# grayhong/self-diagnosing-gan

Measured on AMD Instinct MI355X. Metric: images/sec (G+D step), higher is better.
Workload: dtype f32

## Files before the change

include/diagan_conv_x3.h:

```cpp
#ifndef DIAGAN_CONV_X3_H
#define DIAGAN_CONV_X3_H

#include <stdint.h>

#ifdef __cplusplus
extern "C" {
#endif

int diagan_conv_gemm_set_x3_resident(int mode);
int diagan_conv_gemm_get_x3_resident(void);
int diagan_conv_gemm_last_x3_form(void);
int diagan_conv_gemm_x3_resident_ok(int B, int Hi, int Wi, int Ci, int Ho, int Wo, int Co, int R, int S, int sy, int dr, int off, int up,
                                    int Kp, int pro_mode);

#ifdef __cplusplus
}
#endif
#endif
```

self-diagnosing-gan_amd/csrc/conv_wgrad.hip:

```cpp
#include "conv_common.h"
#include "switches.h"
#include <stdlib.h>
#include <type_traits>


namespace diagan {
bool wgrad_wino_supported(int Hi, int Wi, int Ci, int Ho, int Wo, int Co, int R, int S, int sy, int dr, int off, int up,
                          int Kp);
int wgrad_wino_splits(int B, int Ho, int Wo, int Ci, int Co);
int launch_wgrad_wino(WgradArgs a, int splits, int segments, hipStream_t st);
int launch_wgrad_wino_batched(const WgradArgs* jobs, const int* splits, const int* segments, int n, hipStream_t st);
int wgrad_wino_batch_max();
bool wgrad_x3_takes(const WgradArgs& a, bool x3_on);
int launch_wgrad_x3(const WgradArgs& a, int splits, hipStream_t st);
void wgrad_x3_set(int on);


template <int BNn, int BNk, int PRO, bool P2>
__device__ __forceinline__ void conv_wgrad_body(const WgradArgs& a, const int bid, const int nblk) {
  constexpr int BK = 32;
  constexpr int TM = BNn / 64, TN = BNk / 64;
  constexpr int AC = BNn / 4, BC = BNk / 4;
  constexpr int AJ = BK * AC / 256, BJ = BK * BC / 256;
  constexpr int APR = 256 / AC, BPR = 256 / BC;
  constexpr bool BOX = PRO == PRO_BOX || PRO == PRO_BOX_RELU;
  constexpr int BQ = BOX ? 4 : 1;
  __shared__ __attribute__((aligned(16))) float As[2][BK * BNn];
  __shared__ __attribute__((aligned(16))) float Bs[2][BK * BNk];

  const ConvGeom& g = a.g;
  const int tid = threadIdx.x, lane = tid & 63, wave = tid >> 6;
  const int wm = wave >> 1, wn = wave & 1;
  const int tiles_k = (g.Kp + BNk - 1) / BNk;
  const int logical = xcd_remap(bid, nblk);
  const int split = logical / a.tiles, tile = logical - split * a.tiles;
  const int n0 = (tile / tiles_k) * BNn, k0 = (tile % tiles_k) * BNk;
  const int seg = split / a.splits_per_seg, sub = split - seg * a.splits_per_seg;
  const int step0 = seg * a.seg_steps + sub * a.steps_per_split;
  const int step1 = min(step0 + a.steps_per_split, (seg + 1) * a.seg_steps);

  const int pro_mode = PRO >= 0 ? PRO : a.pro_mode;
  const int ac = tid % AC, ap = tid / AC;
  const int an = n0 + ac * 4;
  const unsigned a_kill = an < g.Co ? 0u : 0x80000000u;
  const int bc = tid % BC, bp = tid / BC;
  const int kf = k0 + bc * 4;
  const int tap = kf / g.Ci, kc = kf - tap * g.Ci;
  const int kr = tap / g.S, ks = tap - kr * g.S;
  const bool b_ok = kf < g.K;
  const int dyo = kr * g.dr + g.off, dxo = ks * g.dr + g.off;
  const int upm = g.up - 1, ush = g.up >> 1;
  const int pstep = (g.Ci * 4) >> ush;
  const int img_bytes = BOX ? (g.Hi - 1) * (g.Wi - 1) * g.Ci * 4 : g.Hi * g.Wi * g.Ci * 4;
  const unsigned ylim = (unsigned)g.Hi << ush, xlim = (unsigned)g.Wi << ush;

  const __amdgpu_buffer_rsrc_t ysrc = __builtin_amdgcn_make_buffer_rsrc(
      const_cast<float*>(a.dy), 0, (int)((unsigned)a.M * g.Co * 4u), 0x00020000);
  const __amdgpu_buffer_rsrc_t xsrc = __builtin_amdgcn_make_buffer_rsrc(
      const_cast<float*>(a.x), 0, (int)((unsigned)g.B * (BOX ? (g.Hi - 1) * (g.Wi - 1) : g.Hi * g.Wi) * g.Ci * 4u), 0x00020000);
  const bool affine = pro_mode == PRO_AFFINE_RELU || pro_mode == PRO_AFFINE;
  f32x4 psc = {1.f, 1.f, 1.f, 1.f}, psh = {0.f, 0.f, 0.f, 0.f};
  if (affine && b_ok) {
    psc = *reinterpret_cast<const f32x4*>(a.pro_scale + kc);
    psh = *reinterpret_cast<const f32x4*>(a.pro_shift + kc);
  }
  int pb[BJ], py[BJ], px[BJ];
#pragma unroll
  for (int j = 0; j < BJ; ++j) {
    const int m = step0 * BK + bp + BPR * j;
    const unsigned t = fdiv((unsigned)m, a.dWo);
    px[j] = m - (int)t * g.Wo;
    const unsigned b = fdiv(t, a.dHo);
    py[j] = (int)t - (int)b * g.Ho;
    pb[j] = (int)b;
  }
  int mstep = step0 * BK;
  unsigned xoff[BJ];
  const unsigned xstep = (unsigned)BK * g.Ci * 4u;
#pragma unroll
  for (int j = 0; j < BJ; ++j)
    xoff[j] = (unsigned)((step0 * BK + bp + BPR * j + dyo * g.Wi + dxo) * g.Ci * 4 + kc * 4);
  unsigned aoff[AJ];
#pragma unroll
  for (int j = 0; j < AJ; ++j) aoff[j] = (((unsigned)(step0 * BK + ap + APR * j)) * g.Co + an) * 4u;
  const unsigned astep = (unsigned)BK * g.Co * 4u;
  f32x4 ra[AJ], rb[BJ * BQ];
  unsigned bmask = 0;
  const bool bias_tile = a.bias_off >= 0 && k0 == 0;
  f32x4 bacc = {0.f, 0.f, 0.f, 0.f};
  auto load_piece = [&](int p) {
    if (p < AJ) {
      ra[p] = __builtin_bit_cast(f32x4, __builtin_amdgcn_raw_buffer_load_b128(ysrc, aoff[p] | a_kill, 0, 0));
      aoff[p] += astep;
      return;
    }
    const int j = p - AJ;
    if (j == 0) bmask = 0;
    if (!BOX && P2 && a.same) {
// ... 444 lines not shown
  DG_REQUIRE(table_dev && n_layers > 0 && total_blocks > 0 && total_blocks < (1L << 31), "wgrad_finish_batched: bad args");
  static_assert(sizeof(WgFinish) == 128, "descriptor layout");
  const WgFinish* tab = (const WgFinish*)table_dev;
  hipStream_t st = (hipStream_t)stream;
  hipLaunchKernelGGL(wgrad_finish_a_kernel, dim3((unsigned)total_blocks), dim3(256), 0, st, tab, n_layers);
  if (any_sn) {
    hipLaunchKernelGGL(wgrad_finish_dot_kernel, dim3(n_layers), dim3(256), 0, st, tab);
    hipLaunchKernelGGL(wgrad_finish_b_kernel, dim3((unsigned)total_blocks), dim3(256), 0, st, tab, n_layers);
  }
  return check_launch("wgrad_finish_batched");
}

static void wgrad_tile(int Co, int Kp, int* bn, int* bk) {
  *bn = Co <= 64 ? 64 : 128;
  *bk = Kp <= 64 ? 64 : 128;
  if (*bn == 128 && *bk == 64) *bn = 64;
}

static void wgrad_gemm_fields(WgradArgs& a, int* bn, int* bk, bool* p2) {
  const ConvGeom& g = a.g;
  wgrad_tile(g.Co, g.Kp, bn, bk);
  a.tiles = cdiv(g.Co, *bn) * cdiv(g.Kp, *bk);
  a.same = (g.Hi == g.Ho && g.Wi == g.Wo && g.sy == 1 && g.up == 1) ? 1 : 0;
  *p2 = (g.Ho & (g.Ho - 1)) == 0 && (g.Wo & (g.Wo - 1)) == 0;
  a.lgW = a.lgHW = 0;
  while ((1 << a.lgW) < g.Wo) ++a.lgW;
  while ((1 << a.lgHW) < g.Ho * g.Wo) ++a.lgHW;
}

static int wgrad_fill_args(WgradArgs& a, const float* dy, const float* x, float* slab, int splits, int segments,
                           int64_t slab_stride, int64_t bias_off, const float* pro_scale, const float* pro_shift, int pro_mode, int B,
                           int Hi, int Wi, int Ci, int Ho, int Wo, int Co, int R, int S, int sy, int dr, int off, int up, int Kp) {
  DG_REQUIRE(dy && x && slab, "conv_wgrad: null tensor");
  DG_REQUIRE(B > 0 && Hi > 0 && Wi > 0 && Ho > 0 && Wo > 0 && R > 0 && S > 0, "conv_wgrad: bad dims");
  DG_REQUIRE(Ci > 0 && (Ci & 3) == 0 && Co > 0 && (Co & 3) == 0, "conv_wgrad: Ci=%d, Co=%d must be multiples of 4", Ci, Co);
  DG_REQUIRE(up == 1 || up == 2, "conv_wgrad: up=%d unsupported", up);
  DG_REQUIRE(dr == 1 || dr == -1, "conv_wgrad: dr must be +-1");
  DG_REQUIRE(Kp % 32 == 0 && Kp >= R * S * Ci, "conv_wgrad: bad Kp=%d", Kp);
  DG_REQUIRE(splits >= 1, "conv_wgrad: splits=%d", splits);
  DG_REQUIRE(pro_mode >= 0 && pro_mode <= PRO_BOX_RELU, "conv_wgrad: bad pro_mode %d", pro_mode);
  DG_REQUIRE(!(pro_mode == PRO_BOX || pro_mode == PRO_BOX_RELU) || (up == 1 && dr == 1 && Hi >= 2 && Wi >= 2),
             "conv_wgrad: the box-sum loader (pro_mode 5 / 6) gathers forward geometries without up-sampling");
  DG_REQUIRE(!(pro_mode == PRO_AFFINE_RELU || pro_mode == PRO_AFFINE) || (pro_scale && pro_shift),
             "conv_wgrad: affine prologue needs scale/shift");
  DG_REQUIRE(slab_stride >= (int64_t)Co * Kp && (bias_off < 0 || bias_off + Co <= slab_stride),
             "conv_wgrad: slab_stride=%ld too small for Co*Kp=%ld (+bias)", (long)slab_stride, (long)Co * Kp);
  DG_REQUIRE((long)Co * Kp * 4 < (1L << 31), "conv_wgrad: weight tensor must be smaller than 2 GiB");
  DG_REQUIRE((long)B * Ho * Wo * Co * 4 < (1L << 31) && (long)B * Hi * Wi * Ci * 4 < (1L << 31),
             "conv_wgrad: tensors must be smaller than 2 GiB (32-bit buffer offsets)");
  a.dy = dy; a.x = x; a.slab = slab; a.pro_scale = pro_scale; a.pro_shift = pro_shift; a.pro_mode = pro_mode;
  a.M = B * Ho * Wo;
  a.g = ConvGeom{B, Hi, Wi, Ci, Ho, Wo, Co, R, S, sy, dr, off, up, R * S * Ci, Kp};
  a.dWo = make_fastdiv((unsigned)Wo);
  a.dHo = make_fastdiv((unsigned)Ho);
  a.adv_b = 32 / (Ho * Wo);
  a.adv_y = (32 % (Ho * Wo)) / Wo;
  a.adv_x = (32 % (Ho * Wo)) % Wo;
  const int total_steps = cdiv(a.M, 32);
  DG_REQUIRE(segments >= 1 && splits % segments == 0, "conv_wgrad: splits=%d not a multiple of segments=%d", splits, segments);
  DG_REQUIRE(segments == 1 || (a.M % (32 * segments)) == 0, "conv_wgrad: %d pixels do not split into %d segments of whole K-steps", a.M, segments);
  a.seg_steps = cdiv(total_steps, segments);
  a.splits_per_seg = splits / segments;
  a.steps_per_split = cdiv(a.seg_steps, a.splits_per_seg);
  a.slab_stride = slab_stride;
  a.bias_off = bias_off;
  return DIAGAN_OK;
}

DIAGAN_API int diagan_conv_wgrad(const float* dy, const float* x, float* slab, int splits, int segments,
                                 int64_t slab_stride, int64_t bias_off, const float* pro_scale, const float* pro_shift, int pro_mode, int B,
                                 int Hi, int Wi, int Ci, int Ho, int Wo, int Co, int R, int S, int sy,
                                 int dr, int off, int up, int Kp, void* stream) {
  WgradArgs a;
  const int rc = wgrad_fill_args(a, dy, x, slab, splits, segments, slab_stride, bias_off, pro_scale, pro_shift, pro_mode, B, Hi, Wi, Ci,
                                 Ho, Wo, Co, R, S, sy, dr, off, up, Kp);
  if (rc != DIAGAN_OK) return rc;
  hipStream_t st = (hipStream_t)stream;
  if (diagan_conv_wgrad_uses_wino(Hi, Wi, Ci, Ho, Wo, Co, R, S, sy, dr, off, up, Kp))
    return launch_wgrad_wino(a, splits, segments, st);
  int bn, bk;
  bool p2;
  wgrad_gemm_fields(a, &bn, &bk, &p2);
  if (bn == 128 && bk == 128 && wgrad_x3_takes(a, diagan_conv_gemm_get_x3b() != 0)) return launch_wgrad_x3(a, splits, st);
  const dim3 grid(a.tiles * splits);
#define DG_WG(BN_, PRO_) do { if (p2) hipLaunchKernelGGL((conv_wgrad_kernel<BN_, 128, PRO_, true>), grid, dim3(256), 0, st, a); \
                              else hipLaunchKernelGGL((conv_wgrad_kernel<BN_, 128, PRO_, false>), grid, dim3(256), 0, st, a); } while (0)
#define DG_WG_ALL(BN_) switch (pro_mode) { \
      case PRO_NONE: DG_WG(BN_, PRO_NONE); break; \
      case PRO_RELU: DG_WG(BN_, PRO_RELU); break; \
      case PRO_AFFINE_RELU: DG_WG(BN_, PRO_AFFINE_RELU); break; \
      case PRO_LRELU: DG_WG(BN_, PRO_LRELU); break; \
      case PRO_BOX: DG_WG(BN_, PRO_BOX); break; \
      case PRO_BOX_RELU: DG_WG(BN_, PRO_BOX_RELU); break; \
      default: DG_WG(BN_, PRO_AFFINE); break; }
  if (bn == 64 && bk == 64) {
    DG_REQUIRE(pro_mode <= PRO_AFFINE, "conv_wgrad: no box-sum loader on the 64 x 64 tile (Kp <= 64)");
    hipLaunchKernelGGL((conv_wgrad_kernel<64, 64>), grid, dim3(256), 0, st, a);
  } else if (bn == 64) {
    DG_WG_ALL(64)
  } else {
    DG_WG_ALL(128)
  }
#undef DG_WG_ALL
#undef DG_WG
  return check_launch("conv_wgrad");
}

struct diagan_wgrad_job {
  const float* dy;
  const float* x;
  float* slab;
  const float* pro_scale;
  const float* pro_shift;
  int64_t slab_stride, bias_off;
  int32_t splits, segments, pro_mode, B, Hi, Wi, Ci, Ho, Wo, Co, R, S, sy, dr, off, up, Kp, pad_;
};
static_assert(sizeof(diagan_wgrad_job) == 128, "diagan_wgrad_job layout");
DIAGAN_API int diagan_conv_wgrad_batch_class(int Hi, int Wi, int Ci, int Ho, int Wo, int Co, int R, int S, int sy, int dr, int off,
                                             int up, int Kp, int pro_mode) {
  if (diagan_conv_wgrad_uses_wino(Hi, Wi, Ci, Ho, Wo, Co, R, S, sy, dr, off, up, Kp)) return 100 + pro_mode;
  int bn, bk;
  wgrad_tile(Co, Kp, &bn, &bk);
  if (bn == 64 && bk == 64) return pro_mode >= PRO_BOX ? 0 : 1000;
  if (pro_mode != PRO_NONE && pro_mode != PRO_RELU && pro_mode != PRO_BOX && pro_mode != PRO_BOX_RELU) return 0;
  const bool p2 = (Ho & (Ho - 1)) == 0 && (Wo & (Wo - 1)) == 0;
  return 2000 + (bn == 128 ? 100 : 0) + 2 * pro_mode + (p2 ? 1 : 0);
}

template <int BN_, int BK_, int PRO_, bool P2_>
static void launch_wgrad_gemm_batched(const WgradBatchArgs& b, int wgs, hipStream_t st) {
  hipLaunchKernelGGL((conv_wgrad_batched_kernel<BN_, BK_, PRO_, P2_>), dim3(wgs), dim3(256), 0, st, b);
}

DIAGAN_API int diagan_conv_wgrad_batched(const diagan_wgrad_job* jobs, int n, void* stream) {
  DG_REQUIRE(jobs && n >= 1 && n <= WG_BATCH_MAX, "conv_wgrad_batched: 1 .. %d jobs", WG_BATCH_MAX);
  WgradArgs a[WG_BATCH_MAX];
  int splits[WG_BATCH_MAX], segments[WG_BATCH_MAX], cls = -1;
  for (int j = 0; j < n; ++j) {
    const diagan_wgrad_job& q = jobs[j];
    const int c = diagan_conv_wgrad_batch_class(q.Hi, q.Wi, q.Ci, q.Ho, q.Wo, q.Co, q.R, q.S, q.sy, q.dr, q.off, q.up, q.Kp, q.pro_mode);
    DG_REQUIRE(c != 0 && (cls < 0 || c == cls), "conv_wgrad_batched: job %d has batch class %d, the launch's is %d "
               "(diagan_conv_wgrad_batch_class: equal non-zero classes share a launch)", j, c, cls);
    cls = c;
    const int rc = wgrad_fill_args(a[j], q.dy, q.x, q.slab, q.splits, q.segments, q.slab_stride, q.bias_off, q.pro_scale, q.pro_shift,
                                   q.pro_mode, q.B, q.Hi, q.Wi, q.Ci, q.Ho, q.Wo, q.Co, q.R, q.S, q.sy, q.dr, q.off, q.up, q.Kp);
    if (rc != DIAGAN_OK) return rc;
    splits[j] = q.splits;
    segments[j] = q.segments;
  }
  hipStream_t st = (hipStream_t)stream;
  if (cls < 1000) return launch_wgrad_wino_batched(a, splits, segments, n, st);
  WgradBatchArgs b;
  b.n = n;
  int wgs = 0, bn = 0, bk = 0;
  bool p2 = false;
  for (int j = 0; j < n; ++j) {
    wgrad_gemm_fields(a[j], &bn, &bk, &p2);
    b.a[j] = a[j];
    b.blk0[j] = wgs;
    b.cnt[j] = a[j].tiles * splits[j];
    wgs += (b.cnt[j] + 7) & ~7;
  }
  for (int j = n; j < WG_BATCH_MAX; ++j) b.blk0[j] = wgs, b.cnt[j] = 0;
  const int pro = jobs[0].pro_mode;
  if (cls == 1000) {
    launch_wgrad_gemm_batched<64, 64, -1, false>(b, wgs, st);
    return check_launch("conv_wgrad_batched");
  }
#define DG_WGB(BN_, PRO_) do { if (p2) launch_wgrad_gemm_batched<BN_, 128, PRO_, true>(b, wgs, st); \
                               else launch_wgrad_gemm_batched<BN_, 128, PRO_, false>(b, wgs, st); } while (0)
#define DG_WGB_ALL(BN_) switch (pro) { \
      case PRO_NONE: DG_WGB(BN_, PRO_NONE); break; \
      case PRO_RELU: DG_WGB(BN_, PRO_RELU); break; \
      case PRO_BOX: DG_WGB(BN_, PRO_BOX); break; \
      default: DG_WGB(BN_, PRO_BOX_RELU); break; }
  if (bn == 128) {
    DG_WGB_ALL(128)
  } else {
    DG_WGB_ALL(64)
  }
#undef DG_WGB_ALL
#undef DG_WGB
  return check_launch("conv_wgrad_batched");
}
DIAGAN_API int diagan_conv_wgrad_batch_max(void) { return WG_BATCH_MAX; }

DIAGAN_API int diagan_conv_wgrad_uses_wino(int Hi, int Wi, int Ci, int Ho, int Wo, int Co, int R, int S, int sy, int dr,
                                           int off, int up, int Kp) {
  return kWino.get(-1, diagan_conv_gemm_get_wino()) && kWinoWgrad.env() &&
         wgrad_wino_supported(Hi, Wi, Ci, Ho, Wo, Co, R, S, sy, dr, off, up, Kp);
}

DIAGAN_API int diagan_conv_wgrad_uses_x3(int B, int Hi, int Wi, int Ci, int Ho, int Wo, int Co, int R, int S, int sy, int dr, int off,
                                         int up, int Kp, int pro_mode, int64_t bias_off) {
  if (B <= 0 || Ho <= 0 || Wo <= 0 || diagan_conv_wgrad_uses_wino(Hi, Wi, Ci, Ho, Wo, Co, R, S, sy, dr, off, up, Kp)) return 0;
  int bn, bk;
  wgrad_tile(Co, Kp, &bn, &bk);
  if (bn != 128 || bk != 128) return 0;
  WgradArgs a;
  a.pro_mode = pro_mode; a.bias_off = bias_off; a.M = B * Ho * Wo;
  a.g = ConvGeom{B, Hi, Wi, Ci, Ho, Wo, Co, R, S, sy, dr, off, up, R * S * Ci, Kp};
  return wgrad_x3_takes(a, diagan_conv_gemm_get_x3b() != 0) ? 1 : 0;
}
DIAGAN_API int diagan_conv_wgrad_set_x3(int on) {
  wgrad_x3_set(on);
  return DIAGAN_OK;
}

DIAGAN_API int diagan_conv_wgrad_splits_geom(int B, int Hi, int Wi, int Ci, int Ho, int Wo, int Co, int R, int S, int sy,
                                             int dr, int off, int up, int Kp) {
  if (diagan_conv_wgrad_uses_wino(Hi, Wi, Ci, Ho, Wo, Co, R, S, sy, dr, off, up, Kp))
    return wgrad_wino_splits(B, Ho, Wo, Ci, Co);
  return diagan_conv_wgrad_splits(B * Ho * Wo, Co, Kp);
}

DIAGAN_API int diagan_conv_wgrad_splits(int M, int Co, int Kp) {
  int bn, bk;
  wgrad_tile(Co, Kp, &bn, &bk);
  const int tiles = cdiv(Co, bn) * cdiv(Kp, bk);
  const int total_steps = cdiv(M, 32);
  const int min_steps = kWgradMinSteps.env();
  const double fixed = kWgradFixed.env();
  int smax = total_steps / min_steps;
  if (smax > 256) smax = 256;
  int splits = 1;
  double best = 1e30;
  const int slots = 512;
  for (int s = 1; s <= smax; ++s) {
    const double t = (double)cdiv(tiles * s, slots) * ((double)total_steps / s + fixed);
    if (t < best * 0.995) { best = t; splits = s; }
  }
  if (splits < 1) splits = 1;
  if (splits > 256) splits = 256;
  return splits;
}

DIAGAN_API int diagan_wgrad_reduce(const float* slab, int splits, int64_t n_elem, float* out, int accumulate,
                                   const float* w, double* dot_partials, void* stream) {
  DG_REQUIRE(slab && out && splits >= 1 && n_elem > 0 && (n_elem & 3) == 0, "wgrad_reduce: bad args");
  const long n4 = n_elem / 4;
  hipLaunchKernelGGL(wgrad_reduce_kernel, dim3(cdiv(n4, 256)), dim3(256), 0, (hipStream_t)stream, slab,
                     splits, n4, out, accumulate, w, dot_partials);
  return check_launch("wgrad_reduce");
}
```

self-diagnosing-gan_amd/csrc/conv_wgrad_x3.hip:

```cpp
#include "conv_common.h"
#include "switches.h"
#include "wino_weights.h"
#include <stdlib.h>

namespace diagan {

constexpr int WX_ROW = 40;
constexpr int WX_PLANE = 128 * WX_ROW;
constexpr int WX_LDS_BYTES = 6 * WX_PLANE * 2;

typedef __bf16 wx_bf16x8 __attribute__((ext_vector_type(8)));

template <bool NOPAD, bool TWO = false>
__global__ __launch_bounds__(256, 2) void conv_wgrad_x3_kernel(const WgradArgs a) {
  extern __shared__ __attribute__((aligned(16))) unsigned short lds[];
  const ConvGeom& g = a.g;
  const int tid = threadIdx.x, lane = tid & 63, wave = __builtin_amdgcn_readfirstlane(tid >> 6);
  const int wm = wave >> 1, wn = wave & 1;
  const int tiles_k = g.Kp >> 7;
  const int logical = xcd_remap(blockIdx.x, gridDim.x);
  const int split = logical / a.tiles, tile = logical - split * a.tiles;
  const int n0 = (tile / tiles_k) * 128, k0 = (tile % tiles_k) * 128;
  const int seg = split / a.splits_per_seg, sub = split - seg * a.splits_per_seg;
  const int step0 = seg * a.seg_steps + sub * a.steps_per_split;
  const int step1 = min(step0 + a.steps_per_split, (seg + 1) * a.seg_steps);

  const int pq = tid & 7, lc = tid >> 3;
  const __amdgpu_buffer_rsrc_t ysrc = __builtin_amdgcn_make_buffer_rsrc(
      const_cast<float*>(a.dy), 0, (int)((unsigned)a.M * g.Co * 4u), 0x00020000);
  const __amdgpu_buffer_rsrc_t xsrc = __builtin_amdgcn_make_buffer_rsrc(
      const_cast<float*>(a.x), 0, (int)((unsigned)g.B * g.Hi * g.Wi * g.Ci * 4u), 0x00020000);
  unsigned aoff = (((unsigned)(step0 * 32 + 4 * pq)) * g.Co + n0 + 4 * lc) * 4u;
  const unsigned astep = 32u * g.Co * 4u;
  const int arow = g.Co * 4;
  const int kf = k0 + 4 * lc;
  const int tap = kf / g.Ci, kc = kf - tap * g.Ci;
  const int kr = tap / g.S, ks = tap - kr * g.S;
  const bool b_ok = kf < g.K;
  const int dyo = kr * g.dr + g.off, dxo = ks * g.dr + g.off;
  const int cb = g.Ci * 4;
  int pb, py, px;
  {
    const int m = step0 * 32 + 4 * pq;
    const unsigned t = fdiv((unsigned)m, a.dWo);
    px = m - (int)t * g.Wo;
    const unsigned b = fdiv(t, a.dHo);
    py = (int)t - (int)b * g.Ho;
    pb = (int)b;
  }
  f32x4 ra[4], rb[4];
  auto load_step = [&]() __attribute__((always_inline)) {
#pragma unroll
    for (int j = 0; j < 4; ++j)
      ra[j] = __builtin_bit_cast(f32x4, __builtin_amdgcn_raw_buffer_load_b128(ysrc, aoff + (unsigned)(j * arow), 0, 0));
    aoff += astep;
    int x = px, y = py, b = pb;
#pragma unroll
    for (int j = 0; j < 4; ++j) {
      const int iy = y * g.sy + dyo, ix = x * g.sy + dxo;
      bool ok = b_ok && b < g.B;
      if (!NOPAD) ok = ok && (unsigned)iy < (unsigned)g.Hi && (unsigned)ix < (unsigned)g.Wi;
      const unsigned off = (unsigned)(((b * g.Hi + iy) * g.Wi + ix) * cb + kc * 4) | (ok ? 0u : 0x80000000u);
      rb[j] = __builtin_bit_cast(f32x4, __builtin_amdgcn_raw_buffer_load_b128(xsrc, off, 0, 0));
      if (j < 3) {
        ++x;
        const int cx = x >= g.Wo ? 1 : 0;
        x = cx ? 0 : x;
        y += cx;
        const int cy = y >= g.Ho ? 1 : 0;
        y = cy ? 0 : y;
        b += cy;
      }
    }
    {
      int x2 = px + a.adv_x, y2 = py + a.adv_y, b2 = pb + a.adv_b;
      const int cx = x2 >= g.Wo ? 1 : 0;
      x2 -= cx ? g.Wo : 0;
      y2 += cx;
      const int cy = y2 >= g.Ho ? 1 : 0;
      y2 -= cy ? g.Ho : 0;
      b2 += cy;
      px = x2; py = y2; pb = b2;
    }
  };
  const int sto = (4 * lc) * WX_ROW + 4 * pq;
  auto store_step = [&]() __attribute__((always_inline)) {
#pragma unroll
    for (int e = 0; e < 4; ++e) {
      u32x2 p0, p1, p2;
      x3_split(f32x4{ra[0][e], ra[1][e], ra[2][e], ra[3][e]}, p0, p1, p2);
      unsigned short* st = lds + sto + e * WX_ROW;
      *reinterpret_cast<u32x2*>(st) = p0;
      *reinterpret_cast<u32x2*>(st + WX_PLANE) = p1;
      if (!TWO) *reinterpret_cast<u32x2*>(st + 2 * WX_PLANE) = p2;
      x3_split(f32x4{rb[0][e], rb[1][e], rb[2][e], rb[3][e]}, p0, p1, p2);
      *reinterpret_cast<u32x2*>(st + 3 * WX_PLANE) = p0;
      *reinterpret_cast<u32x2*>(st + 4 * WX_PLANE) = p1;
      if (!TWO) *reinterpret_cast<u32x2*>(st + 5 * WX_PLANE) = p2;
    }
  };

  f32x16 acc[2][2];
#pragma unroll
  for (int i = 0; i < 2; ++i)
#pragma unroll
    for (int j = 0; j < 2; ++j)
#pragma unroll
      for (int e = 0; e < 16; ++e) acc[i][j][e] = 0.f;
  const int fi = lane & 31, fh = lane >> 5;
  const int fa = (wm * 64 + fi) * WX_ROW, fb = (wn * 64 + fi) * WX_ROW;
  const int oa01 = (fh ? WX_PLANE : 0) + fa, oa02 = (fh ? 2 * WX_PLANE : 0) + fa;
  const int ob00 = 3 * WX_PLANE + fb, ob11 = 4 * WX_PLANE + fb, ob20 = (fh ? 3 : 5) * WX_PLANE + fb;
  wx_bf16x8 fr[2][10];
  auto read_slot = [&](int buf, int sl, int c) __attribute__((always_inline)) {
    const int t = (sl == 2 || sl == 3 || sl == 5 || sl == 8 || sl == 9) ? 32 * WX_ROW : 0;
    const int base = (sl == 0 || sl == 3) ? oa01 : (sl == 6 || sl == 9) ? oa02 : (sl == 1 || sl == 2) ? ob00 : (sl == 4 || sl == 5) ? ob11 : ob20;
    fr[buf][sl] = *reinterpret_cast<const wx_bf16x8*>(lds + base + t + c * 8);
  };
  auto mfmas = [&]() __attribute__((always_inline)) {
#pragma unroll
    for (int sl = 0; sl < (TWO ? 6 : 10); ++sl) read_slot(0, sl, 0);
    __builtin_amdgcn_sched_barrier(0);
    __builtin_amdgcn_s_setprio(1);
#pragma unroll
    for (int c = 0; c < 4; ++c) {
      const int cur = c & 1, nxt = cur ^ 1;
#pragma unroll
      for (int q = 0; q < 12; ++q) {
        const int p = q >> 2, i = (q >> 1) & 1, j = q & 1;
        const int sa = p == 2 ? (i ? 9 : 6) : (i ? 3 : 0);
        const int sb = p == 0 ? 1 + j : (p == 1 ? 4 + j : 7 + j);
        if (TWO && p == 2) continue;
        acc[i][j] = __builtin_amdgcn_mfma_f32_32x32x16_bf16(fr[cur][sa], fr[cur][sb], acc[i][j], 0, 0, 0);
        if (c < 3 && q < (TWO ? 6 : 10)) read_slot(nxt, q, c + 1);
        __builtin_amdgcn_sched_barrier(0);
      }
    }
    __builtin_amdgcn_s_setprio(0);
  };

  if (step0 < step1) {
    load_step();
    store_step();
  }
  __syncthreads();
  for (int step = step0; step < step1; ++step) {
    const bool more = step + 1 < step1;
    if (more) load_step();
    mfmas();
    __syncthreads();
    if (more) {
      store_step();
      __syncthreads();
    }
  }

  float* out = a.slab + (long)split * a.slab_stride;
  const __amdgpu_buffer_rsrc_t osrc = __builtin_amdgcn_make_buffer_rsrc(out, 0, (int)((unsigned)g.Co * g.Kp * 4u), 0x00020000);
  const unsigned rowbytes = (unsigned)g.Kp * 4u;
#pragma unroll
  for (int i = 0; i < 2; ++i)
#pragma unroll
    for (int j = 0; j < 2; ++j) {
      const int k = k0 + wn * 64 + j * 32 + fi;
      const int nrow = n0 + wm * 64 + i * 32 + 4 * fh;
      const unsigned vbase = ((unsigned)nrow * g.Kp + k) * 4u;
#pragma unroll
      for (int e = 0; e < 16; ++e)
        __builtin_amdgcn_raw_buffer_store_b32(__float_as_uint(acc[i][j][e]), osrc, vbase, (int)(((e & 3) + 8 * (e >> 2)) * rowbytes), 0);
    }
}

static int wgrad_x3_switch = -1;
void wgrad_x3_set(int on) { wgrad_x3_switch = on; }
static bool wgrad_x3_enabled() { return kWgradX3.get(-1, wgrad_x3_switch) != 0; }

bool wgrad_x3_takes(const WgradArgs& a, bool x3_on) {
  const ConvGeom& g = a.g;
  if (!x3_on || !wgrad_x3_enabled()) return false;
  if (a.pro_mode != PRO_NONE || a.bias_off >= 0 || g.up != 1) return false;
  if ((g.Co & 127) || (g.Kp & 127) || g.K != g.Kp || (g.Ci & 31)) return false;
  if (wgrad_x3_switch == 2) return true;
  return (double)a.M * g.Co * g.K >= kWgradX3MinMac.env();
}

static bool wgrad_x3_nopad(const ConvGeom& g) {
  const int lo = g.dr > 0 ? g.off : g.off - (g.R - 1), hi_y = (g.Ho - 1) * g.sy + (g.dr > 0 ? g.off + g.R - 1 : g.off);
  const int lo_x = g.dr > 0 ? g.off : g.off - (g.S - 1), hi_x = (g.Wo - 1) * g.sy + (g.dr > 0 ? g.off + g.S - 1 : g.off);
  return lo >= 0 && lo_x >= 0 && hi_y < g.Hi && hi_x < g.Wi;
}

int x3_pieces();

int launch_wgrad_x3(const WgradArgs& a, int splits, hipStream_t st) {
  static FuncAttrLatch l0, l1, m0, m1;
  const dim3 grid(a.tiles * splits);
  if (x3_pieces() == 2) {
    if (wgrad_x3_nopad(a.g)) {
      DG_LDS(m1, (conv_wgrad_x3_kernel<true, true>), WX_LDS_BYTES);
      hipLaunchKernelGGL((conv_wgrad_x3_kernel<true, true>), grid, dim3(256), WX_LDS_BYTES, st, a);
    } else {
      DG_LDS(m0, (conv_wgrad_x3_kernel<false, true>), WX_LDS_BYTES);
      hipLaunchKernelGGL((conv_wgrad_x3_kernel<false, true>), grid, dim3(256), WX_LDS_BYTES, st, a);
    }
    return check_launch("conv_wgrad_x3 (two pieces)");
  }
  if (wgrad_x3_nopad(a.g)) {
    DG_LDS(l1, conv_wgrad_x3_kernel<true>, WX_LDS_BYTES);
    hipLaunchKernelGGL((conv_wgrad_x3_kernel<true>), grid, dim3(256), WX_LDS_BYTES, st, a);
  } else {
    DG_LDS(l0, conv_wgrad_x3_kernel<false>, WX_LDS_BYTES);
    hipLaunchKernelGGL((conv_wgrad_x3_kernel<false>), grid, dim3(256), WX_LDS_BYTES, st, a);
  }
  return check_launch("conv_wgrad_x3");
}

}
```

self-diagnosing-gan_amd/diagan/ops/conv.py:

```python
import torch

from diagan import _native as nat

PRO_NONE, PRO_RELU, PRO_AFFINE_RELU, PRO_LRELU, PRO_AFFINE = 0, 1, 2, 3, 4
PRO_BOX, PRO_BOX_RELU = 5, 6
TILE_SHAPES = {1: (128, 128, 2, 2, 32, False), 2: (128, 64, 2, 2, 32, False), 3: (64, 64, 2, 2, 32, False),
               4: (128, 64, 4, 1, 32, False), 5: (256, 64, 4, 1, 32, False), 6: (64, 64, 2, 2, 64, False),
               7: (64, 64, 2, 2, 32, True), 8: (128, 64, 2, 2, 32, True), 14: (64, 64, 2, 2, 32, True)}


def gemm_kernel_name(cfg, mode, Co=128, w4pool=False, Ci=0, RS=9, mapped=False):
    if cfg in (11, 12) and w4pool:
        return f"conv_wino4_kernel<{mode if cfg == 11 else 0},{cfg - 10},false>"
    if cfg == 9:
        return f"conv_wino_kernel<{mode}>"
    if cfg in (13, 15):
        x3 = "true" if (nat.fn("diagan_conv_gemm_get_wino4x")() > 0 and Ci % 32 == 0) else "false"
        return f"conv_wino4_kernel<{mode},{0 if cfg == 13 else 3},{x3}>"
    if cfg == 11:
        return f"conv_wino_pool_kernel<{mode},false,{2 if Co % 128 == 0 else 1}>"
    if cfg == 12:
        return f"conv_wino_pool_kernel<0,true,{2 if Co % 128 == 0 else 1}>"
    if cfg == 17:
        return f"conv_gemm_x3b_kernel<{mode},{'true' if mapped else 'false'}>"
# ... 132 lines not shown
    nat.call("diagan_conv_gemm_set_wino4x", -1 if mode is None else (1 if mode else 0))


def set_winograd4(mode):
    nat.call("diagan_conv_gemm_set_wino4", -1 if mode is None else (2 if mode == 'force-pool' else (1 if mode else 0)))


def round_up(x, m):
    return (x + m - 1) // m * m


class Geom:

    def __init__(self, kind, Ci, Co, R, S, stride=1, pad=0):
        assert kind in ('conv', 'convT')
        self.kind, self.Ci, self.Co, self.R, self.S, self.stride, self.pad = kind, Ci, Co, R, S, stride, pad
        self.Kp = round_up(R * S * Ci, 32)
        self.Kd = round_up(R * S * Co, 32)

    def out_hw(self, Hi, Wi):
        if self.kind == 'conv':
            return ((Hi + 2 * self.pad - self.R) // self.stride + 1,
                    (Wi + 2 * self.pad - self.S) // self.stride + 1)
        return ((Hi - 1) * self.stride - 2 * self.pad + self.R, (Wi - 1) * self.stride - 2 * self.pad + self.S)

    def fwd_params(self):
        return (self.stride, 1, -self.pad, 1) if self.kind == 'conv' else (1, -1, self.pad, self.stride)

    def dgrad_params(self):
        return (1, -1, self.pad, self.stride) if self.kind == 'conv' else (self.stride, 1, -self.pad, 1)

    def abi_fwd(self, B, Hi, Wi, out_hw=None):
        Ho, Wo = self.out_hw(Hi, Wi) if out_hw is None else out_hw
        return (B, Hi, Wi, self.Ci, Ho, Wo, self.Co, self.R, self.S) + self.fwd_params() + (self.Kp,)

    def abi_dgrad(self, B, Hi, Wi):
        Ho, Wo = self.out_hw(Hi, Wi)
        return (B, Ho, Wo, self.Co, Hi, Wi, self.Ci, self.R, self.S) + self.dgrad_params() + (self.Kd,)


def _pro3(pro):
    if pro is None:
        return PRO_NONE, None, None
    if len(pro) > 3 and pro[3]:
        raise RuntimeError("grouped BatchNorm prologues exist for the forward kernels only")
    return tuple(pro)[:3]


def set_gemm_x3(on):
    nat.call("diagan_conv_gemm_set_x3", -1 if on is None else (1 if on else 0))
    nat.call("diagan_conv_gemm_set_x3b", -1 if on is None else (1 if on else 0))


def set_gemm_x3_resident(on):
    from diagan._native import conv_x3_abi as xnat
    xnat.call("diagan_conv_gemm_set_x3_resident", -1 if on is None else (1 if on else 0))


def last_x3_form():
    from diagan._native import conv_x3_abi as xnat
    return xnat.fn("diagan_conv_gemm_last_x3_form")()


def gemm_x3_resident_ok(geom, B, Hi, Wi, dgrad=False, mode=PRO_NONE):
    from diagan._native import conv_x3_abi as xnat
    geo = geom.abi_dgrad(B, Hi, Wi) if dgrad else geom.abi_fwd(B, Hi, Wi)
    return bool(xnat.fn("diagan_conv_gemm_x3_resident_ok")(*geo, mode))


def set_gemm_x3b(on):
    nat.call("diagan_conv_gemm_set_x3b", -1 if on is None else (1 if on else 0))


def set_x3_pieces(n):
    nat.call("diagan_conv_gemm_set_x3_pieces", 0 if n is None else int(n))


def set_wgrad_x3(on):
    nat.call("diagan_conv_wgrad_set_x3", -1 if on is None else (int(on) if on else 0))


def wgrad_uses_x3(geom, B, Hi, Wi, Ho, Wo, mode=0, bias_off=-1):
    return bool(nat.fn("diagan_conv_wgrad_uses_x3")(*geom.abi_fwd(B, Hi, Wi, (Ho, Wo)), mode, bias_off))


_TICKETS = {}


def set_splitk_fused(on):
    nat.call("diagan_conv_gemm_set_splitk_fused", -1 if on is None else (1 if on else 0))
    if on:
        dev = torch.cuda.current_device()
        if dev not in _TICKETS:
            _TICKETS[dev] = torch.zeros(1 << 16, dtype=torch.int32, device=torch.device('cuda', dev))
        nat.call("diagan_conv_gemm_set_splitk_tickets", _TICKETS[dev].data_ptr(), _TICKETS[dev].numel())
    else:
        nat.call("diagan_conv_gemm_set_splitk_tickets", None, 0)


class ConvOpts(_ct.Structure):
    _fields_ = [(n, _ct.c_int32) for n in ("wino", "wino4", "wino4x", "gemm_x3", "gemm_x3b", "splitk_fused", "force_ksplit", "tune")] + \
               [("tickets", _ct.c_void_p), ("ticket_slots", _ct.c_int64), ("gemm_x3_resident", _ct.c_int32)]


def next_opts(tickets=None, **fields):
    o = ConvOpts(-1, -1, -1, -1, -1, -1, 0, -1, None, 0, -1)
    for k, v in fields.items():
        setattr(o, k, int(v))
    if tickets is not None:
        o.tickets, o.ticket_slots = tickets.data_ptr(), tickets.numel()
    nat.call("diagan_conv_gemm_next_opts", _ct.byref(o))


def pending_opts():
    o = ConvOpts()
    nat.call("diagan_conv_gemm_pending_opts", _ct.byref(o))
    return o


def _opts_key(o):
    return tuple(getattr(o, n) for n, _ in ConvOpts._fields_[:8]) + (o.gemm_x3_resident,)


def _without_wino(o):
    m = ConvOpts.from_buffer_copy(o)
    m.wino, m.wino4 = 0, 0
    return m


def last_cfg():
    return nat.fn("diagan_conv_gemm_last_cfg")()


def wg_x_shape(x, pro):
    B, H, W, Ci = x.shape
    if pro is not None and int(pro[0]) >= PRO_BOX:
        return B, H + 1, W + 1, Ci
    return B, H, W, Ci


def _chk(t, name):
    if t is None:
        return
    if not (t.is_cuda and t.dtype == torch.float32 and t.is_contiguous()):
        raise RuntimeError(f"{name}: expected a contiguous CUDA float32 tensor, got "
                           f"{t.dtype} {t.device} contiguous={t.is_contiguous()}")


def _gemm(x, w, out, geo_params, R, S, Kp, bias, residual, mask_src, mask_slope, pro, out_scale, tile_cfg,
          res_relu=False, row_scale=None, want_stats=False, wino=True, res_up=False, pool=False, unpool=False, up_in=False,
          wsite=None, wversion=None, res_unpool=False, out_map=None):
    B, Hi, Wi, Ci = x.shape
    _, Ho, Wo, Co = out.shape
    if out_map is not None:
        Ho, Wo = out_map[9], out_map[10]
    if up_in:
        Hi, Wi, tile_cfg = 2 * Hi, 2 * Wi, 15
        if pool or unpool or mask_src is not None:
            raise RuntimeError("conv_gemm: the up-sampled-input launch takes no pooling and no backward mask")
    if unpool:
        Hi, Wi, tile_cfg = 2 * Hi, 2 * Wi, 12
    if pool:
        Ho, Wo, tile_cfg = 2 * Ho, 2 * Wo, 11
        if want_stats or res_up or mask_src is not None:
            raise RuntimeError("conv_gemm: the pooled launch takes no statistics, mask or half-resolution residual")
    mode, scale, shift, group_imgs = (tuple(pro) + (0,))[:4] if pro is not None else (PRO_NONE, None, None, 0)
# ... 451 lines not shown
```

Baseline: 5372.

## Route box-sum and bias-column weight gradients through the bf16 x3 MFMA kernel

New measurement: 5396 (median of 6 runs). Within noise of the previous version (+0.4%).

```diff
diff --git a/include/diagan_conv_x3.h b/include/diagan_conv_x3.h
--- a/include/diagan_conv_x3.h
+++ b/include/diagan_conv_x3.h
@@ -13,6 +13,11 @@
 int diagan_conv_gemm_x3_resident_ok(int B, int Hi, int Wi, int Ci, int Ho, int Wo, int Co, int R, int S, int sy, int dr, int off, int up,
                                     int Kp, int pro_mode);
 
+int diagan_conv_wgrad_set_x3_box(int mode);
+int diagan_conv_wgrad_get_x3_box(void);
+int diagan_conv_wgrad_box_uses_x3(int B, int Hi, int Wi, int Ci, int Ho, int Wo, int Co, int R, int S, int sy, int dr, int off, int up,
+                                  int Kp, int pro_mode, int64_t bias_off);
+
 #ifdef __cplusplus
 }
 #endif
diff --git a/self-diagnosing-gan_amd/csrc/conv_wgrad.hip b/self-diagnosing-gan_amd/csrc/conv_wgrad.hip
--- a/self-diagnosing-gan_amd/csrc/conv_wgrad.hip
+++ b/self-diagnosing-gan_amd/csrc/conv_wgrad.hip
@@ -14,6 +14,8 @@
 bool wgrad_x3_takes(const WgradArgs& a, bool x3_on);
 int launch_wgrad_x3(const WgradArgs& a, int splits, hipStream_t st);
 void wgrad_x3_set(int on);
+bool wgrad_x3_box_takes(const WgradArgs& a, bool x3_on);
+int launch_wgrad_x3_box_batched(const WgradBatchArgs& b, int wgs, int pro_mode, hipStream_t st);
 
 
 template <int BNn, int BNk, int PRO, bool P2>
@@ -624,6 +626,7 @@
   bool p2;
   wgrad_gemm_fields(a, &bn, &bk, &p2);
   if (bn == 128 && bk == 128 && wgrad_x3_takes(a, diagan_conv_gemm_get_x3b() != 0)) return launch_wgrad_x3(a, splits, st);
+  if (bn == 128 && bk == 128 && wgrad_x3_box_takes(a, diagan_conv_gemm_get_x3b() != 0)) return launch_wgrad_x3(a, splits, st);
   const dim3 grid(a.tiles * splits);
 #define DG_WG(BN_, PRO_) do { if (p2) hipLaunchKernelGGL((conv_wgrad_kernel<BN_, 128, PRO_, true>), grid, dim3(256), 0, st, a); \
                               else hipLaunchKernelGGL((conv_wgrad_kernel<BN_, 128, PRO_, false>), grid, dim3(256), 0, st, a); } while (0)
@@ -716,6 +719,30 @@
       case PRO_RELU: DG_WGB(BN_, PRO_RELU); break; \
       case PRO_BOX: DG_WGB(BN_, PRO_BOX); break; \
       default: DG_WGB(BN_, PRO_BOX_RELU); break; }
+  if (bn == 128 && (pro >= PRO_BOX || pro == PRO_NONE)) {
+    const bool x3_on = diagan_conv_gemm_get_x3b() != 0;
+    WgradBatchArgs bx, bf;
+    int wx = 0, wf = 0;
+    bx.n = bf.n = 0;
+    for (int j = 0; j < n; ++j) {
+      const bool x3 = bk == 128 && wgrad_x3_box_takes(b.a[j], x3_on);
+      WgradBatchArgs& t = x3 ? bx : bf;
+      int& w = x3 ? wx : wf;
+      t.a[t.n] = b.a[j];
+      t.blk0[t.n] = w;
+      t.cnt[t.n] = b.cnt[j];
+      w += (b.cnt[j] + 7) & ~7;
+      ++t.n;
+    }
+    for (int j = bx.n; j < WG_BATCH_MAX; ++j) bx.blk0[j] = wx, bx.cnt[j] = 0;
+    for (int j = bf.n; j < WG_BATCH_MAX; ++j) bf.blk0[j] = wf, bf.cnt[j] = 0;
+    if (bx.n > 0) {
+      const int rc = launch_wgrad_x3_box_batched(bx, wx, pro, st);
+      if (rc != DIAGAN_OK || bf.n == 0) return rc;
+      b = bf;
+      wgs = wf;
+    }
+  }
   if (bn == 128) {
     DG_WGB_ALL(128)
   } else {
@@ -743,6 +770,17 @@
   a.pro_mode = pro_mode; a.bias_off = bias_off; a.M = B * Ho * Wo;
   a.g = ConvGeom{B, Hi, Wi, Ci, Ho, Wo, Co, R, S, sy, dr, off, up, R * S * Ci, Kp};
   return wgrad_x3_takes(a, diagan_conv_gemm_get_x3b() != 0) ? 1 : 0;
+}
+DIAGAN_API int diagan_conv_wgrad_box_uses_x3(int B, int Hi, int Wi, int Ci, int Ho, int Wo, int Co, int R, int S, int sy, int dr, int off,
+                                             int up, int Kp, int pro_mode, int64_t bias_off) {
+  if (B <= 0 || Ho <= 0 || Wo <= 0 || diagan_conv_wgrad_uses_wino(Hi, Wi, Ci, Ho, Wo, Co, R, S, sy, dr, off, up, Kp)) return 0;
+  int bn, bk;
+  wgrad_tile(Co, Kp, &bn, &bk);
+  if (bn != 128 || bk != 128) return 0;
+  WgradArgs a;
+  a.pro_mode = pro_mode; a.bias_off = bias_off; a.M = B * Ho * Wo;
+  a.g = ConvGeom{B, Hi, Wi, Ci, Ho, Wo, Co, R, S, sy, dr, off, up, R * S * Ci, Kp};
+  return wgrad_x3_box_takes(a, diagan_conv_gemm_get_x3b() != 0) ? 1 : 0;
 }
 DIAGAN_API int diagan_conv_wgrad_set_x3(int on) {
   wgrad_x3_set(on);
diff --git a/self-diagnosing-gan_amd/csrc/conv_wgrad_x3.hip b/self-diagnosing-gan_amd/csrc/conv_wgrad_x3.hip
--- a/self-diagnosing-gan_amd/csrc/conv_wgrad_x3.hip
+++ b/self-diagnosing-gan_amd/csrc/conv_wgrad_x3.hip
@@ -11,14 +11,23 @@
 
 typedef __bf16 wx_bf16x8 __attribute__((ext_vector_type(8)));
 
-template <bool NOPAD, bool TWO = false>
-__global__ __launch_bounds__(256, 2) void conv_wgrad_x3_kernel(const WgradArgs a) {
-  extern __shared__ __attribute__((aligned(16))) unsigned short lds[];
+__device__ __forceinline__ float pq_sum(float v) {
+  v += __builtin_bit_cast(float, __builtin_amdgcn_update_dpp(0, __builtin_bit_cast(int, v), 0xB1, 0xF, 0xF, true));
+  v += __builtin_bit_cast(float, __builtin_amdgcn_update_dpp(0, __builtin_bit_cast(int, v), 0x4E, 0xF, 0xF, true));
+  v += __builtin_bit_cast(float, __builtin_amdgcn_update_dpp(0, __builtin_bit_cast(int, v), 0x141, 0xF, 0xF, true));
+  return v;
+}
+
+template <bool NOPAD, bool TWO, int PRO, bool BIAS = false>
+__device__ __forceinline__ void conv_wgrad_x3_body(const WgradArgs& a, const int bid, const int nblk, unsigned short* lds) {
+  constexpr bool BOX = PRO == PRO_BOX || PRO == PRO_BOX_RELU;
+  constexpr int BQ = BOX ? 4 : 1;
+  static_assert(!(BOX && (NOPAD || TWO)), "the box-sum loader tests every load and serves the three-piece kernel only");
   const ConvGeom& g = a.g;
   const int tid = threadIdx.x, lane = tid & 63, wave = __builtin_amdgcn_readfirstlane(tid >> 6);
   const int wm = wave >> 1, wn = wave & 1;
   const int tiles_k = g.Kp >> 7;
-  const int logical = xcd_remap(blockIdx.x, gridDim.x);
+  const int logical = xcd_remap(bid, nblk);
   const int split = logical / a.tiles, tile = logical - split * a.tiles;
   const int n0 = (tile / tiles_k) * 128, k0 = (tile % tiles_k) * 128;
   const int seg = split / a.splits_per_seg, sub = split - seg * a.splits_per_seg;
@@ -29,7 +38,7 @@
   const __amdgpu_buffer_rsrc_t ysrc = __builtin_amdgcn_make_buffer_rsrc(
       const_cast<float*>(a.dy), 0, (int)((unsigned)a.M * g.Co * 4u), 0x00020000);
   const __amdgpu_buffer_rsrc_t xsrc = __builtin_amdgcn_make_buffer_rsrc(
-      const_cast<float*>(a.x), 0, (int)((unsigned)g.B * g.Hi * g.Wi * g.Ci * 4u), 0x00020000);
+      const_cast<float*>(a.x), 0, (int)((unsigned)g.B * (BOX ? (g.Hi - 1) * (g.Wi - 1) : g.Hi * g.Wi) * g.Ci * 4u), 0x00020000);
   unsigned aoff = (((unsigned)(step0 * 32 + 4 * pq)) * g.Co + n0 + 4 * lc) * 4u;
   const unsigned astep = 32u * g.Co * 4u;
   const int arow = g.Co * 4;
@@ -48,7 +57,10 @@
     py = (int)t - (int)b * g.Ho;
     pb = (int)b;
   }
-  f32x4 ra[4], rb[4];
+  f32x4 ra[4], rb[4 * BQ];
+  constexpr bool BIAS_ON = BOX || BIAS;
+  const bool bias_tile = BIAS_ON && a.bias_off >= 0 && k0 == 0;
+  f32x4 bacc = {0.f, 0.f, 0.f, 0.f};
   auto load_step = [&]() __attribute__((always_inline)) {
 #pragma unroll
     for (int j = 0; j < 4; ++j)
@@ -58,10 +70,22 @@
 #pragma unroll
     for (int j = 0; j < 4; ++j) {
       const int iy = y * g.sy + dyo, ix = x * g.sy + dxo;
+      if constexpr (BOX) {
+        const int H = g.Hi - 1, W = g.Wi - 1;
+        const bool okp = b_ok && b < g.B;
+#pragma unroll
+        for (int q = 0; q < 4; ++q) {
+          const int yy = iy - 1 + (q >> 1), xx = ix - 1 + (q & 1);
+          const bool ok = okp && (unsigned)yy < (unsigned)H && (unsigned)xx < (unsigned)W;
+          const unsigned off = (unsigned)(((b * H + yy) * W + xx) * cb + kc * 4) | (ok ? 0u : 0x80000000u);
+          rb[j * 4 + q] = __builtin_bit_cast(f32x4, __builtin_amdgcn_raw_buffer_load_b128(xsrc, off, 0, 0));
+        }
+      } else {
       bool ok = b_ok && b < g.B;
       if (!NOPAD) ok = ok && (unsigned)iy < (unsigned)g.Hi && (unsigned)ix < (unsigned)g.Wi;
       const unsigned off = (unsigned)(((b * g.Hi + iy) * g.Wi + ix) * cb + kc * 4) | (ok ? 0u : 0x80000000u);
       rb[j] = __builtin_bit_cast(f32x4, __builtin_amdgcn_raw_buffer_load_b128(xsrc, off, 0, 0));
+      }
       if (j < 3) {
         ++x;
         const int cx = x >= g.Wo ? 1 : 0;
@@ -85,6 +109,31 @@
   };
   const int sto = (4 * lc) * WX_ROW + 4 * pq;
   auto store_step = [&]() __attribute__((always_inline)) {
+    if constexpr (BOX) {
+#pragma unroll
+      for (int j = 0; j < 4; ++j) {
+        f32x4 sum = {0.f, 0.f, 0.f, 0.f};
+#pragma unroll
+        for (int q = 0; q < 4; ++q) {
+          f32x4 t = rb[j * 4 + q];
+          if (PRO == PRO_BOX_RELU) {
+#pragma unroll
+            for (int e = 0; e < 4; ++e) t[e] = fmaxf(t[e], 0.f);
+          }
+          sum += t;
+        }
+        rb[j] = sum * 0.25f;
+      }
+    }
+    if constexpr (BIAS_ON) {
+      if (bias_tile) {
+        f32x4 t = ra[0];
+#pragma unroll
+        for (int j = 1; j < 4; ++j) t += ra[j];
+#pragma unroll
+        for (int e = 0; e < 4; ++e) bacc[e] += pq_sum(t[e]);
+      }
+    }
 #pragma unroll
     for (int e = 0; e < 4; ++e) {
       u32x2 p0, p1, p2;
@@ -156,6 +205,10 @@
   }
 
   float* out = a.slab + (long)split * a.slab_stride;
+  if (bias_tile && pq == 0) {
+#pragma unroll
+    for (int e = 0; e < 4; ++e) out[a.bias_off + n0 + 4 * lc + e] = bacc[e];
+  }
   const __amdgpu_buffer_rsrc_t osrc = __builtin_amdgcn_make_buffer_rsrc(out, 0, (int)((unsigned)g.Co * g.Kp * 4u), 0x00020000);
   const unsigned rowbytes = (unsigned)g.Kp * 4u;
 #pragma unroll
@@ -171,9 +224,29 @@
     }
 }
 
+template <bool NOPAD, bool TWO = false, int PRO = PRO_NONE, bool BIAS = false>
+__global__ __launch_bounds__(256, 2) void conv_wgrad_x3_kernel(const WgradArgs a) {
+  extern __shared__ __attribute__((aligned(16))) unsigned short lds[];
+  conv_wgrad_x3_body<NOPAD, TWO, PRO, BIAS>(a, blockIdx.x, gridDim.x, lds);
+}
+
+template <int PRO>
+__global__ __launch_bounds__(256, 2) void conv_wgrad_x3_batched_kernel(const WgradBatchArgs b) {
+  extern __shared__ __attribute__((aligned(16))) unsigned short lds[];
+  int j = 0;
+  while (j + 1 < b.n && (int)blockIdx.x >= b.blk0[j + 1]) ++j;
+  j = __builtin_amdgcn_readfirstlane(j);
+  const int local = (int)blockIdx.x - b.blk0[j];
+  if (local >= b.cnt[j]) return;
+  const WgradArgs a = b.a[j];
+  conv_wgrad_x3_body<false, false, PRO, true>(a, local, b.cnt[j], lds);
+}
+
 static int wgrad_x3_switch = -1;
 void wgrad_x3_set(int on) { wgrad_x3_switch = on; }
 static bool wgrad_x3_enabled() { return kWgradX3.get(-1, wgrad_x3_switch) != 0; }
+
+int x3_pieces();
 
 bool wgrad_x3_takes(const WgradArgs& a, bool x3_on) {
   const ConvGeom& g = a.g;
@@ -184,17 +257,46 @@
   return (double)a.M * g.Co * g.K >= kWgradX3MinMac.env();
 }
 
+static int g_wgrad_x3_box = -1;
+static Switch kWgradX3Box{{"DIAGAN_WGRAD_X3_BOX", 1}};
+static SwitchF kWgradX3BoxMinMac{"DIAGAN_WGRAD_X3_BOX_MIN_MAC", 1.2e9};
+void wgrad_x3_box_set(int mode) { g_wgrad_x3_box = mode; }
+bool wgrad_x3_box_on() { return kWgradX3Box.get(-1, g_wgrad_x3_box) != 0; }
+
+bool wgrad_x3_box_takes(const WgradArgs& a, bool x3_on) {
+  const ConvGeom& g = a.g;
+  if (!x3_on || !wgrad_x3_enabled() || !wgrad_x3_box_on() || x3_pieces() == 2) return false;
+  const bool box = a.pro_mode == PRO_BOX || a.pro_mode == PRO_BOX_RELU;
+  if (!(box || (a.pro_mode == PRO_NONE && a.bias_off >= 0)) || g.up != 1) return false;
+  if ((g.Co & 127) || (g.Kp & 127) || g.K != g.Kp || (g.Ci & 31)) return false;
+  if (wgrad_x3_switch == 2) return true;
+  return (double)a.M * g.Co * g.K >= kWgradX3BoxMinMac.env();
+}
+
 static bool wgrad_x3_nopad(const ConvGeom& g) {
   const int lo = g.dr > 0 ? g.off : g.off - (g.R - 1), hi_y = (g.Ho - 1) * g.sy + (g.dr > 0 ? g.off + g.R - 1 : g.off);
   const int lo_x = g.dr > 0 ? g.off : g.off - (g.S - 1), hi_x = (g.Wo - 1) * g.sy + (g.dr > 0 ? g.off + g.S - 1 : g.off);
   return lo >= 0 && lo_x >= 0 && hi_y < g.Hi && hi_x < g.Wi;
 }
 
-int x3_pieces();
-
 int launch_wgrad_x3(const WgradArgs& a, int splits, hipStream_t st) {
-  static FuncAttrLatch l0, l1, m0, m1;
+  static FuncAttrLatch l0, l1, m0, m1, b5, b6, b0;
   const dim3 grid(a.tiles * splits);
+  if (a.pro_mode == PRO_NONE && a.bias_off >= 0) {
+    DG_LDS(b0, (conv_wgrad_x3_kernel<false, false, PRO_NONE, true>), WX_LDS_BYTES);
+    hipLaunchKernelGGL((conv_wgrad_x3_kernel<false, false, PRO_NONE, true>), grid, dim3(256), WX_LDS_BYTES, st, a);
+    return check_launch("conv_wgrad_x3 (bias column)");
+  }
+  if (a.pro_mode == PRO_BOX) {
+    DG_LDS(b5, (conv_wgrad_x3_kernel<false, false, PRO_BOX>), WX_LDS_BYTES);
+    hipLaunchKernelGGL((conv_wgrad_x3_kernel<false, false, PRO_BOX>), grid, dim3(256), WX_LDS_BYTES, st, a);
+    return check_launch("conv_wgrad_x3 (box sums)");
+  }
+  if (a.pro_mode == PRO_BOX_RELU) {
+    DG_LDS(b6, (conv_wgrad_x3_kernel<false, false, PRO_BOX_RELU>), WX_LDS_BYTES);
+    hipLaunchKernelGGL((conv_wgrad_x3_kernel<false, false, PRO_BOX_RELU>), grid, dim3(256), WX_LDS_BYTES, st, a);
+    return check_launch("conv_wgrad_x3 (box sums)");
+  }
   if (x3_pieces() == 2) {
     if (wgrad_x3_nopad(a.g)) {
       DG_LDS(m1, (conv_wgrad_x3_kernel<true, true>), WX_LDS_BYTES);
@@ -215,4 +317,28 @@
   return check_launch("conv_wgrad_x3");
 }
 
-}
+int launch_wgrad_x3_box_batched(const WgradBatchArgs& b, int wgs, int pro_mode, hipStream_t st) {
+  static FuncAttrLatch b5, b6, b0;
+  if (pro_mode == PRO_NONE) {
+    DG_LDS(b0, conv_wgrad_x3_batched_kernel<PRO_NONE>, WX_LDS_BYTES);
+    hipLaunchKernelGGL(conv_wgrad_x3_batched_kernel<PRO_NONE>, dim3(wgs), dim3(256), WX_LDS_BYTES, st, b);
+  } else if (pro_mode == PRO_BOX) {
+    DG_LDS(b5, conv_wgrad_x3_batched_kernel<PRO_BOX>, WX_LDS_BYTES);
+    hipLaunchKernelGGL(conv_wgrad_x3_batched_kernel<PRO_BOX>, dim3(wgs), dim3(256), WX_LDS_BYTES, st, b);
+  } else {
+    DG_LDS(b6, conv_wgrad_x3_batched_kernel<PRO_BOX_RELU>, WX_LDS_BYTES);
+    hipLaunchKernelGGL(conv_wgrad_x3_batched_kernel<PRO_BOX_RELU>, dim3(wgs), dim3(256), WX_LDS_BYTES, st, b);
+  }
+  return check_launch("conv_wgrad_x3_batched (box sums)");
+}
+
+}
+
+using namespace diagan;
+
+DIAGAN_API int diagan_conv_wgrad_set_x3_box(int mode) {
+  DG_REQUIRE(mode >= -1 && mode <= 1, "set_x3_box: -1, 0 or 1");
+  wgrad_x3_box_set(mode);
+  return DIAGAN_OK;
+}
+DIAGAN_API int diagan_conv_wgrad_get_x3_box(void) { return wgrad_x3_box_on() ? 1 : 0; }
diff --git a/self-diagnosing-gan_amd/diagan/ops/conv.py b/self-diagnosing-gan_amd/diagan/ops/conv.py
--- a/self-diagnosing-gan_amd/diagan/ops/conv.py
+++ b/self-diagnosing-gan_amd/diagan/ops/conv.py
@@ -238,6 +238,16 @@
 
 def wgrad_uses_x3(geom, B, Hi, Wi, Ho, Wo, mode=0, bias_off=-1):
     return bool(nat.fn("diagan_conv_wgrad_uses_x3")(*geom.abi_fwd(B, Hi, Wi, (Ho, Wo)), mode, bias_off))
+
+
+def set_wgrad_x3_box(on):
+    from diagan._native import conv_x3_abi as xnat
+    xnat.call("diagan_conv_wgrad_set_x3_box", -1 if on is None else (1 if on else 0))
+
+
+def wgrad_box_uses_x3(geom, B, Hi, Wi, Ho, Wo, mode=PRO_BOX, bias_off=-1):
+    from diagan._native import conv_x3_abi as xnat
+    return bool(xnat.fn("diagan_conv_wgrad_box_uses_x3")(*geom.abi_fwd(B, Hi, Wi, (Ho, Wo)), mode, bias_off))
 
 
 _TICKETS = {}
```
